# Hxyou/MSCLIP

Hardware: AMD Instinct MI355X
Metric: image-text pairs/sec ViT-B/32 bf16 (higher is better)
Workload: dtype bf16; 1 GPU; MS-CLIP-S b32-yfcc-msclips fwd + contrastive step (both towers, gather, logits, symmetric CE), per-GPU batch 512, 224x224 images + 77-token captions, random-init weights; per_gpu_batch=512, global_batch=512, parallelism=dp1, bn=eval (folded running statistics), rccl_ranks=1

## Files before the change

msclip_amd/csrc/attention.hip:

```cpp
#include <stdlib.h>
#include "common.h"
#include "plan.h"
#include "../../include/msclip_hip.h"

namespace {

template <int NT, bool CAUSAL, int WPB>
__global__ __launch_bounds__(WPB * 64) void attn_kernel(const bf16_t* __restrict__ qkv, bf16_t* __restrict__ out,
                                                   int nsamples, int Lfix, int H, int ldq, int ldo,
                                                   const int* __restrict__ cu, int pad_rows, const int* __restrict__ dims) {
  constexpr int KP = NT * 32;
  constexpr int KPS = KP + 8;
  extern __shared__ __attribute__((aligned(16))) bf16_t vt_all[];

  const int lane = threadIdx.x & 63;
  const int wave = __builtin_amdgcn_readfirstlane(threadIdx.x >> 6);
  const int pair = blockIdx.x * WPB + wave;
  if (pair >= nsamples * H) {
    const int r = pair - nsamples * H;
    if (dims) pad_rows = min(pad_rows, dims[4]);
    if (cu && r < pad_rows) {
      bf16_t* orow = out + (size_t)(cu[nsamples] + r) * ldo;
      for (int c = lane * 8; c < H * 64; c += 512) *(uint4*)(orow + c) = make_uint4(0, 0, 0, 0);
    }
    return;
  }
  const int b = pair / H, h = pair - b * H;
  bf16_t* vt = vt_all + wave * (64 * KPS);

  const int c0 = cu ? __builtin_amdgcn_readfirstlane(cu[b]) : b * Lfix;
  const int L = cu ? min(__builtin_amdgcn_readfirstlane(cu[b + 1]) - c0, KP) : Lfix;
  const size_t row0 = (size_t)c0;
  const bf16_t* qbase = qkv + row0 * ldq + h * 64;
  const bf16_t* kbase = qbase + H * 64;
  const bf16_t* vbase = qbase + 2 * H * 64;

  const int fr = lane & 31, fhi = lane >> 5;

  if constexpr (NT <= 3) {
    constexpr int NVI = KP / 8;
    uint4 vreg[NVI];
    {
      const int c = lane & 7;
#pragma unroll
      for (int i = 0; i < NVI; ++i) {
        const int key = i * 8 + (lane >> 3);
        vreg[i] = key < L ? *(const uint4*)(vbase + (size_t)key * ldq + c * 8) : make_uint4(0, 0, 0, 0);
      }
    }
    bf16x8 qf[NT][4], kf[NT][4];
#pragma unroll
    for (int t = 0; t < NT; ++t) {
      const int row = min(t * 32 + fr, L - 1);
      if (t * 32 < L) {
#pragma unroll
        for (int kk = 0; kk < 4; ++kk) {
          qf[t][kk] = *(const bf16x8*)(qbase + (size_t)row * ldq + (kk * 2 + fhi) * 8);
          kf[t][kk] = *(const bf16x8*)(kbase + (size_t)row * ldq + (kk * 2 + fhi) * 8);
        }
      } else {
#pragma unroll
        for (int kk = 0; kk < 4; ++kk) qf[t][kk] = kf[t][kk] = bf16x8{};
      }
    }
    {
      const int c = lane & 7;
#pragma unroll
      for (int i = 0; i < NVI; ++i) {
        const int key = i * 8 + (lane >> 3);
        const int w = key & 15;
        const int slot = (key & ~15) + (((w >> 2) & 1) << 3) + (w & 3) + ((w >> 3) << 2);
        bf16_t* dst = vt + (c * 8) * KPS + slot;
        const uint4 u = vreg[i];
        dst[0 * KPS] = (bf16_t)(u.x & 0xffff); dst[1 * KPS] = (bf16_t)(u.x >> 16);
        dst[2 * KPS] = (bf16_t)(u.y & 0xffff); dst[3 * KPS] = (bf16_t)(u.y >> 16);
        dst[4 * KPS] = (bf16_t)(u.z & 0xffff); dst[5 * KPS] = (bf16_t)(u.z >> 16);
        dst[6 * KPS] = (bf16_t)(u.w & 0xffff); dst[7 * KPS] = (bf16_t)(u.w >> 16);
      }
    }
    __builtin_amdgcn_wave_barrier();

#pragma unroll
    for (int qt = 0; qt < NT; ++qt) {
      if (qt * 32 < L) {
        const int nkt = CAUSAL ? (qt + 1) : NT;
        f32x16 s[NT];
#pragma unroll
        for (int kt = 0; kt < NT; ++kt) {
#pragma unroll
          for (int r = 0; r < 16; ++r) s[kt][r] = 0.f;
          if (kt < nkt && kt * 32 < L) {
#pragma unroll
            for (int kk = 0; kk < 4; ++kk)
              s[kt] = __builtin_amdgcn_mfma_f32_32x32x16_bf16(kf[kt][kk], qf[qt][kk], s[kt], 0, 0, 0);
          }
        }
        const int q = qt * 32 + fr;
        float mx = -INFINITY;
#pragma unroll
        for (int kt = 0; kt < NT; ++kt)
          if (kt < nkt) {
#pragma unroll
            for (int r = 0; r < 16; ++r) {
              const int key = kt * 32 + (r & 3) + 8 * (r >> 2) + 4 * fhi;
              const bool ok = key < L && (!CAUSAL || key <= q);
              s[kt][r] = ok ? s[kt][r] : -INFINITY;
              mx = fmaxf(mx, s[kt][r]);
            }
          }
        mx = fmaxf(mx, __shfl_xor(mx, 32, 64));
        float sum = 0.f;
#pragma unroll
        for (int kt = 0; kt < NT; ++kt)
          if (kt < nkt) {
#pragma unroll
            for (int r = 0; r < 16; ++r) {
              const float p = __expf(s[kt][r] - mx);
              s[kt][r] = p;
              sum += p;
            }
          }
        sum += __shfl_xor(sum, 32, 64);
        const float inv = 1.f / sum;
        f32x16 o[2];
#pragma unroll
        for (int dt = 0; dt < 2; ++dt)
#pragma unroll
          for (int r = 0; r < 16; ++r) o[dt][r] = 0.f;
#pragma unroll
        for (int kt = 0; kt < NT; ++kt) {
          if (kt < nkt && kt * 32 < L) {
#pragma unroll
            for (int half = 0; half < 2; ++half) {
              bf16x8 pf;
#pragma unroll
              for (int e = 0; e < 8; ++e) pf[e] = (__bf16)s[kt][half * 8 + e];
              const int st = kt * 2 + half;
#pragma unroll
              for (int dt = 0; dt < 2; ++dt) {
                const bf16x8 vf = *(const bf16x8*)(vt + (dt * 32 + fr) * KPS + st * 16 + fhi * 8);
                o[dt] = __builtin_amdgcn_mfma_f32_32x32x16_bf16(vf, pf, o[dt], 0, 0, 0);
              }
            }
          }
        }
        {
          bf16_t* orow = out + (row0 + min(q, L - 1)) * ldo + h * 64;
#pragma unroll
          for (int dt = 0; dt < 2; ++dt) {
            unsigned pk[4][2];
#pragma unroll
            for (int g = 0; g < 4; ++g) {
              pk[g][0] = pack_bf16x2(o[dt][g * 4 + 0] * inv, o[dt][g * 4 + 1] * inv);
              pk[g][1] = pack_bf16x2(o[dt][g * 4 + 2] * inv, o[dt][g * 4 + 3] * inv);
            }
#pragma unroll
            for (int s2 = 0; s2 < 2; ++s2) {
              const auto x = __builtin_amdgcn_permlane32_swap(pk[2 * s2][0], pk[2 * s2 + 1][0], false, false);
              const auto y = __builtin_amdgcn_permlane32_swap(pk[2 * s2][1], pk[2 * s2 + 1][1], false, false);
              if (q < L) *(uint4*)(orow + dt * 32 + s2 * 16 + fhi * 8) = make_uint4(x[0], y[0], x[1], y[1]);
            }
          }
        }
      }
    }
    return;
  }

  {
    const int c = lane & 7;
#pragma unroll 2
    for (int k0 = 0; k0 < KP; k0 += 8) {
      const int key = k0 + (lane >> 3);
      uint4 u = make_uint4(0, 0, 0, 0);
      if (key < L) u = *(const uint4*)(vbase + (size_t)key * ldq + c * 8);
      const int w = key & 15;
      const int slot = (key & ~15) + (((w >> 2) & 1) << 3) + (w & 3) + ((w >> 3) << 2);
      bf16_t* dst = vt + (c * 8) * KPS + slot;
      dst[0 * KPS] = (bf16_t)(u.x & 0xffff); dst[1 * KPS] = (bf16_t)(u.x >> 16);
      dst[2 * KPS] = (bf16_t)(u.y & 0xffff); dst[3 * KPS] = (bf16_t)(u.y >> 16);
      dst[4 * KPS] = (bf16_t)(u.z & 0xffff); dst[5 * KPS] = (bf16_t)(u.z >> 16);
      dst[6 * KPS] = (bf16_t)(u.w & 0xffff); dst[7 * KPS] = (bf16_t)(u.w >> 16);
    }
  }
  __builtin_amdgcn_s_waitcnt(0xc07f);
  __builtin_amdgcn_wave_barrier();

  for (int qt = 0; qt < NT; ++qt) {
    if (qt * 32 >= L) break;
    const int qrow = min(qt * 32 + fr, L - 1);
    bf16x8 qf[4];
#pragma unroll
    for (int kk = 0; kk < 4; ++kk) qf[kk] = *(const bf16x8*)(qbase + (size_t)qrow * ldq + (kk * 2 + fhi) * 8);

    const int nkt = CAUSAL ? (qt + 1) : NT;
    f32x16 s[NT];
#pragma unroll
    for (int kt = 0; kt < NT; ++kt) {
#pragma unroll
      for (int r = 0; r < 16; ++r) s[kt][r] = 0.f;
      if (kt < nkt && kt * 32 < L) {
        const int krow = min(kt * 32 + fr, L - 1);
#pragma unroll
        for (int kk = 0; kk < 4; ++kk) {
          const bf16x8 kf = *(const bf16x8*)(kbase + (size_t)krow * ldq + (kk * 2 + fhi) * 8);
          s[kt] = __builtin_amdgcn_mfma_f32_32x32x16_bf16(kf, qf[kk], s[kt], 0, 0, 0);
        }
      }
    }

    const int q = qt * 32 + fr;
    float mx = -INFINITY;
#pragma unroll
    for (int kt = 0; kt < NT; ++kt)
#pragma unroll
      for (int r = 0; r < 16; ++r) {
        const int key = kt * 32 + (r & 3) + 8 * (r >> 2) + 4 * fhi;
        const bool ok = key < L && (!CAUSAL || key <= q) && kt < nkt;
        s[kt][r] = ok ? s[kt][r] : -INFINITY;
        mx = fmaxf(mx, s[kt][r]);
      }
    mx = fmaxf(mx, __shfl_xor(mx, 32, 64));
    float sum = 0.f;
#pragma unroll
    for (int kt = 0; kt < NT; ++kt)
#pragma unroll
      for (int r = 0; r < 16; ++r) {
        const float p = __expf(s[kt][r] - mx);
        s[kt][r] = p;
        sum += p;
      }
    sum += __shfl_xor(sum, 32, 64);
    const float inv = 1.f / sum;

    f32x16 o[2];
#pragma unroll
    for (int dt = 0; dt < 2; ++dt)
#pragma unroll
      for (int r = 0; r < 16; ++r) o[dt][r] = 0.f;
#pragma unroll
    for (int kt = 0; kt < NT; ++kt) {
      if (kt < nkt && kt * 32 < L) {
#pragma unroll
        for (int half = 0; half < 2; ++half) {
          bf16x8 pf;
#pragma unroll
          for (int e = 0; e < 8; ++e) pf[e] = (__bf16)s[kt][half * 8 + e];
          const int st = kt * 2 + half;
#pragma unroll
          for (int dt = 0; dt < 2; ++dt) {
            const bf16x8 vf = *(const bf16x8*)(vt + (dt * 32 + fr) * KPS + st * 16 + fhi * 8);
            o[dt] = __builtin_amdgcn_mfma_f32_32x32x16_bf16(vf, pf, o[dt], 0, 0, 0);
          }
        }
      }
    }

    if (q < L) {
      bf16_t* orow = out + (row0 + q) * ldo + h * 64;
#pragma unroll
      for (int dt = 0; dt < 2; ++dt)
#pragma unroll
        for (int g = 0; g < 4; ++g) {
          uint2 v;
          v.x = pack_bf16x2(o[dt][g * 4 + 0] * inv, o[dt][g * 4 + 1] * inv);
          v.y = pack_bf16x2(o[dt][g * 4 + 2] * inv, o[dt][g * 4 + 3] * inv);
          *(uint2*)(orow + dt * 32 + g * 8 + fhi * 4) = v;
        }
    }
  }
}

template <int NT, bool CAUSAL>
__global__ __launch_bounds__(256, 2) void attn_wg_kernel(const bf16_t* __restrict__ qkv, bf16_t* __restrict__ out,
                                                      int nsamples, int L, int H, int ldq, int ldo) {
  constexpr int KP = NT * 32;
  constexpr int KPS = KP + 8;
  constexpr int KROW = 72;
  __shared__ __attribute__((aligned(16))) bf16_t kl[KP * KROW];
  __shared__ __attribute__((aligned(16))) bf16_t vt[64 * KPS];

  const int tid = threadIdx.x, lane = tid & 63;
  const int wave = __builtin_amdgcn_readfirstlane(tid >> 6);
  const int pair = blockIdx.x;
  const int b = pair / H, h = pair - b * H;
  const size_t row0 = (size_t)b * L;
  const bf16_t* qbase = qkv + row0 * ldq + h * 64;
  const bf16_t* kbase = qbase + H * 64;
  const bf16_t* vbase = qbase + 2 * H * 64;
  const int fr = lane & 31, fhi = lane >> 5;

  auto load_q = [&](int qt, bf16x8 (&qf)[4]) {
    const int qrow = min(qt * 32 + fr, L - 1);
#pragma unroll
    for (int kk = 0; kk < 4; ++kk) {
      const bf16_t* p = qbase + (size_t)qrow * ldq + (kk * 2 + fhi) * 8;
      asm volatile("global_load_dwordx4 %0, %1, off" : "=&v"(qf[kk]) : "v"(p));
    }
  };
  bf16x8 qcur[4], qnext[4];
#pragma unroll
  for (int kk = 0; kk < 4; ++kk) qcur[kk] = qnext[kk] = bf16x8{};
  if (wave * 32 < L) load_q(wave, qcur);

  {
    const int c = tid & 7;
    uint4 ku[NT], vu[NT];
#pragma unroll
    for (int i = 0; i < NT; ++i) {
      const int key = (tid >> 3) + 32 * i;
      const int kc = min(key, L - 1);
      ku[i] = *(const uint4*)(kbase + (size_t)kc * ldq + c * 8);
      vu[i] = *(const uint4*)(vbase + (size_t)kc * ldq + c * 8);
    }
#pragma unroll
    for (int i = 0; i < NT; ++i)
      if ((tid >> 3) + 32 * i >= L) ku[i] = vu[i] = make_uint4(0, 0, 0, 0);
#pragma unroll
    for (int i = 0; i < NT; ++i) {
      const int key = (tid >> 3) + 32 * i;
      *(uint4*)(kl + key * KROW + c * 8) = ku[i];
      const int w = key & 15;
      const int slot = (key & ~15) + (((w >> 2) & 1) << 3) + (w & 3) + ((w >> 3) << 2);
      bf16_t* dst = vt + (c * 8) * KPS + slot;
      dst[0 * KPS] = (bf16_t)(vu[i].x & 0xffff); dst[1 * KPS] = (bf16_t)(vu[i].x >> 16);
      dst[2 * KPS] = (bf16_t)(vu[i].y & 0xffff); dst[3 * KPS] = (bf16_t)(vu[i].y >> 16);
      dst[4 * KPS] = (bf16_t)(vu[i].z & 0xffff); dst[5 * KPS] = (bf16_t)(vu[i].z >> 16);
      dst[6 * KPS] = (bf16_t)(vu[i].w & 0xffff); dst[7 * KPS] = (bf16_t)(vu[i].w >> 16);
    }
  }
  asm volatile("s_waitcnt vmcnt(0)" : "+v"(qcur[0]), "+v"(qcur[1]), "+v"(qcur[2]), "+v"(qcur[3])::"memory");
  __syncthreads();

  for (int qt = wave; qt < NT && qt * 32 < L; qt += 4) {
    const bool more = (qt + 4) < NT && (qt + 4) * 32 < L;
    if (more) load_q(qt + 4, qnext);
    const int nkt = CAUSAL ? (qt + 1) : NT;
    f32x16 s[NT];
    if constexpr (!CAUSAL) {
      bf16x8 kf[2][4];
#pragma unroll
      for (int kk = 0; kk < 4; ++kk) kf[0][kk] = *(const bf16x8*)(kl + fr * KROW + (kk * 2 + fhi) * 8);
#pragma unroll
      for (int kt = 0; kt < NT; ++kt) {
        if (kt + 1 < NT) {
#pragma unroll
          for (int kk = 0; kk < 4; ++kk)
            kf[(kt + 1) & 1][kk] = *(const bf16x8*)(kl + ((kt + 1) * 32 + fr) * KROW + (kk * 2 + fhi) * 8);
        }
#pragma unroll
        for (int r = 0; r < 16; ++r) s[kt][r] = 0.f;
        __builtin_amdgcn_sched_barrier(0);
#pragma unroll
        for (int kk = 0; kk < 4; ++kk) s[kt] = __builtin_amdgcn_mfma_f32_32x32x16_bf16(kf[kt & 1][kk], qcur[kk], s[kt], 0, 0, 0);
        __builtin_amdgcn_sched_barrier(0);
      }
    } else {
#pragma unroll
      for (int kt = 0; kt < NT; ++kt) {
#pragma unroll
        for (int r = 0; r < 16; ++r) s[kt][r] = 0.f;
        if (kt < nkt && kt * 32 < L) {
#pragma unroll
          for (int kk = 0; kk < 4; ++kk) {
            const bf16x8 kf = *(const bf16x8*)(kl + (kt * 32 + fr) * KROW + (kk * 2 + fhi) * 8);
            s[kt] = __builtin_amdgcn_mfma_f32_32x32x16_bf16(kf, qcur[kk], s[kt], 0, 0, 0);
          }
        }
      }
    }
    const int q = qt * 32 + fr;
    float mx = -INFINITY;
#pragma unroll
    for (int kt = 0; kt < NT; ++kt) {
      const bool inside = kt * 32 + 32 <= L && (!CAUSAL || kt < qt) && kt < nkt;
      if (inside) {
#pragma unroll
        for (int r = 0; r < 16; ++r) mx = fmaxf(mx, s[kt][r]);
      } else {
#pragma unroll
        for (int r = 0; r < 16; ++r) {
          const int key = kt * 32 + (r & 3) + 8 * (r >> 2) + 4 * fhi;
          const bool ok = key < L && (!CAUSAL || key <= q) && kt < nkt;
          s[kt][r] = ok ? s[kt][r] : -INFINITY;
          mx = fmaxf(mx, s[kt][r]);
        }
      }
    }
    mx = fmaxf(mx, __shfl_xor(mx, 32, 64));
    const float mxl = mx * 1.44269504f;
    float sum = 0.f;
#pragma unroll
    for (int kt = 0; kt < NT; ++kt)
#pragma unroll
      for (int r = 0; r < 16; ++r) {
        const float p = __builtin_amdgcn_exp2f(fmaf(s[kt][r], 1.44269504f, -mxl));
        s[kt][r] = p;
        sum += p;
      }
    sum += __shfl_xor(sum, 32, 64);
    const float inv = 1.f / sum;
    f32x16 o[2];
#pragma unroll
    for (int dt = 0; dt < 2; ++dt)
#pragma unroll
      for (int r = 0; r < 16; ++r) o[dt][r] = 0.f;
    if constexpr (!CAUSAL) {
      bf16x8 vf[2][2];
#pragma unroll
      for (int dt = 0; dt < 2; ++dt) vf[0][dt] = *(const bf16x8*)(vt + (dt * 32 + fr) * KPS + fhi * 8);
#pragma unroll
      for (int st = 0; st < 2 * NT; ++st) {
        if (st + 1 < 2 * NT) {
#pragma unroll
          for (int dt = 0; dt < 2; ++dt)
            vf[(st + 1) & 1][dt] = *(const bf16x8*)(vt + (dt * 32 + fr) * KPS + (st + 1) * 16 + fhi * 8);
        }
        bf16x8 pf;
#pragma unroll
        for (int e = 0; e < 8; ++e) pf[e] = (__bf16)s[st >> 1][(st & 1) * 8 + e];
        __builtin_amdgcn_sched_barrier(0);
#pragma unroll
        for (int dt = 0; dt < 2; ++dt) o[dt] = __builtin_amdgcn_mfma_f32_32x32x16_bf16(vf[st & 1][dt], pf, o[dt], 0, 0, 0);
        __builtin_amdgcn_sched_barrier(0);
      }
    } else {
#pragma unroll
      for (int kt = 0; kt < NT; ++kt) {
        if (kt < nkt && kt * 32 < L) {
#pragma unroll
          for (int half = 0; half < 2; ++half) {
            bf16x8 pf;
#pragma unroll
            for (int e = 0; e < 8; ++e) pf[e] = (__bf16)s[kt][half * 8 + e];
            const int st = kt * 2 + half;
#pragma unroll
            for (int dt = 0; dt < 2; ++dt) {
              const bf16x8 vf = *(const bf16x8*)(vt + (dt * 32 + fr) * KPS + st * 16 + fhi * 8);
              o[dt] = __builtin_amdgcn_mfma_f32_32x32x16_bf16(vf, pf, o[dt], 0, 0, 0);
            }
          }
        }
      }
    }
    {
      bf16_t* orow = out + (row0 + min(q, L - 1)) * ldo + h * 64;
#pragma unroll
      for (int dt = 0; dt < 2; ++dt) {
        unsigned pk[4][2];
#pragma unroll
        for (int g = 0; g < 4; ++g) {
          pk[g][0] = pack_bf16x2(o[dt][g * 4 + 0] * inv, o[dt][g * 4 + 1] * inv);
          pk[g][1] = pack_bf16x2(o[dt][g * 4 + 2] * inv, o[dt][g * 4 + 3] * inv);
        }
#pragma unroll
        for (int s2 = 0; s2 < 2; ++s2) {
          const auto x = __builtin_amdgcn_permlane32_swap(pk[2 * s2][0], pk[2 * s2 + 1][0], false, false);
          const auto y = __builtin_amdgcn_permlane32_swap(pk[2 * s2][1], pk[2 * s2 + 1][1], false, false);
          if (q < L) *(uint4*)(orow + dt * 32 + s2 * 16 + fhi * 8) = make_uint4(x[0], y[0], x[1], y[1]);
        }
      }
    }
    if (more) {
      asm volatile("s_waitcnt vmcnt(4)" : "+v"(qnext[0]), "+v"(qnext[1]), "+v"(qnext[2]), "+v"(qnext[3])::"memory");
#pragma unroll
      for (int kk = 0; kk < 4; ++kk) qcur[kk] = qnext[kk];
    }
  }
}

template <int NT>
int launch_wg(const void* qkv, void* out, int nsamples, int L, int H, int ldq, int ldo, int causal, hipStream_t st) {
  const int pairs = nsamples * H;
  if (causal)
    hipLaunchKernelGGL((attn_wg_kernel<NT, true>), dim3(pairs), dim3(256), 0, st, (const bf16_t*)qkv, (bf16_t*)out,
                       nsamples, L, H, ldq, ldo);
  else
    hipLaunchKernelGGL((attn_wg_kernel<NT, false>), dim3(pairs), dim3(256), 0, st, (const bf16_t*)qkv, (bf16_t*)out,
                       nsamples, L, H, ldq, ldo);
  return msclip_launch_status();
}

template <int MAXI>
__global__ __launch_bounds__(256) void attn_lastq_kernel(const bf16_t* __restrict__ qc, int ldqc, const bf16_t* __restrict__ kv,
                                                    int ldkv, bf16_t* __restrict__ out, int ldo, int nsamples, int L, int H,
                                                    const int* __restrict__ last_row, int row_base, const int* __restrict__ cu) {
  const int lane = threadIdx.x & 63;
  const int pair = blockIdx.x * 4 + (threadIdx.x >> 6);
  if (pair >= nsamples * H) return;
  const int b = pair / H, h = pair - b * H;
  const int row0 = row_base + (cu ? cu[b] : b * L);
  int nk = cu ? cu[b + 1] - cu[b] : (last_row ? last_row[b] - row0 + 1 : L);
  nk = min(max(nk, 1), L);
  const int g = lane >> 3, c = lane & 7;
  const bf16_t* kbase = kv + (size_t)row0 * ldkv + H * 64 + h * 64 + c * 8;
  const bf16_t* vbase = kbase + H * 64;
  float q8[8];
  unpack_bf16x8(*(const uint4*)(qc + (size_t)b * ldqc + h * 64 + c * 8), q8);
  float s[MAXI];
  float m = -INFINITY;
#pragma unroll
  for (int i = 0; i < MAXI; ++i) {
    const int key = i * 8 + g;
    float d = 0.f;
    if (key < nk) {
      float kf[8];
      unpack_bf16x8(*(const uint4*)(kbase + (size_t)key * ldkv), kf);
#pragma unroll
      for (int e = 0; e < 8; ++e) d = fmaf(q8[e], kf[e], d);
    }
    d += __shfl_xor(d, 1, 64);
    d += __shfl_xor(d, 2, 64);
    d += __shfl_xor(d, 4, 64);
    s[i] = key < nk ? d : -INFINITY;
    m = fmaxf(m, s[i]);
  }
  m = fmaxf(m, __shfl_xor(m, 8, 64));
  m = fmaxf(m, __shfl_xor(m, 16, 64));
  m = fmaxf(m, __shfl_xor(m, 32, 64));
  float sum = 0.f;
#pragma unroll
  for (int i = 0; i < MAXI; ++i) {
    const float p = i * 8 + g < nk ? __expf(s[i] - m) : 0.f;
    sum += p;
    s[i] = bf16_to_f32(f32_to_bf16(p));
  }
  sum += __shfl_xor(sum, 8, 64);
  sum += __shfl_xor(sum, 16, 64);
  sum += __shfl_xor(sum, 32, 64);
  float acc[8] = {0.f, 0.f, 0.f, 0.f, 0.f, 0.f, 0.f, 0.f};
#pragma unroll
  for (int i = 0; i < MAXI; ++i) {
    const int key = i * 8 + g;
    if (key < nk) {
      float vf[8];
      unpack_bf16x8(*(const uint4*)(vbase + (size_t)key * ldkv), vf);
#pragma unroll
      for (int e = 0; e < 8; ++e) acc[e] = fmaf(s[i], vf[e], acc[e]);
    }
  }
#pragma unroll
  for (int e = 0; e < 8; ++e) {
    acc[e] += __shfl_xor(acc[e], 8, 64);
    acc[e] += __shfl_xor(acc[e], 16, 64);
    acc[e] += __shfl_xor(acc[e], 32, 64);
  }
  if (g == 0) {
    const float r = 1.f / sum;
    uint4 o;
    o.x = pack_bf16x2(acc[0] * r, acc[1] * r);
    o.y = pack_bf16x2(acc[2] * r, acc[3] * r);
    o.z = pack_bf16x2(acc[4] * r, acc[5] * r);
    o.w = pack_bf16x2(acc[6] * r, acc[7] * r);
    *(uint4*)(out + (size_t)b * ldo + h * 64 + c * 8) = o;
  }
}

template <int NT>
int launch(const void* qkv, void* out, int nsamples, int L, int H, int ldq, int ldo, int causal, hipStream_t st,
           const int* cu = nullptr, int pad_rows = 0, const int* dims = nullptr) {
  constexpr int WPB = NT > 4 ? 2 : 4;
  const int pairs = nsamples * H + (cu ? pad_rows : 0);
  const int grid = (pairs + WPB - 1) / WPB;
  const size_t lds = WPB * 64 * (NT * 32 + 8) * sizeof(bf16_t);
  if (causal)
    hipLaunchKernelGGL((attn_kernel<NT, true, WPB>), dim3(grid), dim3(WPB * 64), lds, st, (const bf16_t*)qkv,
                       (bf16_t*)out, nsamples, L, H, ldq, ldo, cu, pad_rows, dims);
  else
    hipLaunchKernelGGL((attn_kernel<NT, false, WPB>), dim3(grid), dim3(WPB * 64), lds, st, (const bf16_t*)qkv,
                       (bf16_t*)out, nsamples, L, H, ldq, ldo, cu, pad_rows, dims);
  return msclip_launch_status();
}

}

extern "C" int msclip_attention(const void* qkv, void* out, int nsamples, int L, int heads, int ldq, int ldo,
                                int causal, void* stream) {
  MSCLIP_PLAN_HOOK(msclip_attention, stream, qkv, out, nsamples, L, heads, ldq, ldo, causal);
  if (!qkv || !out || nsamples <= 0 || L <= 0 || heads <= 0 || (ldq % 8) || (ldo % 8)) return MSCLIP_EINVAL;
  hipStream_t st = (hipStream_t)stream;
  if (L <= 64) return launch<2>(qkv, out, nsamples, L, heads, ldq, ldo, causal, st);
  if (L <= 96) return launch<3>(qkv, out, nsamples, L, heads, ldq, ldo, causal, st);
  if (L <= 224) {
    const char* old = getenv("MSCLIP_ATTN_WAVE");
    if (old && old[0] == '1') return launch<7>(qkv, out, nsamples, L, heads, ldq, ldo, causal, st);
    return launch_wg<7>(qkv, out, nsamples, L, heads, ldq, ldo, causal, st);
  }
  if (L <= 288) return launch_wg<9>(qkv, out, nsamples, L, heads, ldq, ldo, causal, st);
  return MSCLIP_EINVAL;
}

static int lastq_launch(const void* q, int ldqc, const void* qkv, int ldq, void* out, int ldo, int nsamples, int L, int heads,
                        const int* last_row, int row_base, const int* cu, void* stream) {
  if (!q || !qkv || !out || nsamples <= 0 || L <= 0 || L > 288 || heads <= 0 || (ldqc % 8) || (ldq % 8) || (ldo % 8) || ldo < heads * 64 || row_base < 0)
    return MSCLIP_EINVAL;
  const int grid = (nsamples * heads + 3) / 4;
  hipStream_t st = (hipStream_t)stream;
#define LASTQ(MAXI)                                                                                                            \
  hipLaunchKernelGGL(attn_lastq_kernel<MAXI>, dim3(grid), dim3(256), 0, st, (const bf16_t*)q, ldqc, (const bf16_t*)qkv, ldq,   \
                     (bf16_t*)out, ldo, nsamples, L, heads, last_row, row_base, cu)
  if (L <= 32) LASTQ(4);
  else if (L <= 64) LASTQ(8);
  else if (L <= 80) LASTQ(10);
  else if (L <= 128) LASTQ(16);
  else if (L <= 256) LASTQ(32);
  else LASTQ(36);
#undef LASTQ
  return msclip_launch_status();
}

extern "C" int msclip_attention_lastq(const void* q, int ldqc, const void* qkv, int ldq, void* out, int ldo, int nsamples, int L,
                                      int heads, const int* last_row, int row_base, void* stream) {
  MSCLIP_PLAN_HOOK(msclip_attention_lastq, stream, q, ldqc, qkv, ldq, out, ldo, nsamples, L, heads, last_row, row_base);
  return lastq_launch(q, ldqc, qkv, ldq, out, ldo, nsamples, L, heads, last_row, row_base, nullptr, stream);
}

extern "C" int msclip_attention_lastq_varlen(const void* q, int ldqc, const void* qkv, int ldq, void* out, int ldo, int nsamples,
                                             int Lmax, int heads, const int* cu, int row_base, void* stream) {
  MSCLIP_PLAN_HOOK(msclip_attention_lastq_varlen, stream, q, ldqc, qkv, ldq, out, ldo, nsamples, Lmax, heads, cu, row_base);
  if (!cu) return MSCLIP_EINVAL;
  return lastq_launch(q, ldqc, qkv, ldq, out, ldo, nsamples, Lmax, heads, nullptr, row_base, cu, stream);
}

extern "C" int msclip_attention_varlen(const void* qkv, void* out, const int* cu, int nsamples, int Lmax, int heads, int ldq,
                                       int ldo, int causal, int pad_rows, const int* dims, void* stream) {
  MSCLIP_PLAN_HOOK(msclip_attention_varlen, stream, qkv, out, cu, nsamples, Lmax, heads, ldq, ldo, causal, pad_rows, dims);
  if (!qkv || !out || !cu || nsamples <= 0 || Lmax <= 0 || Lmax > 96 || heads <= 0 || (ldq % 8) || (ldo % 8) || pad_rows < 0 ||
      pad_rows > 255)
    return MSCLIP_EINVAL;
  hipStream_t st = (hipStream_t)stream;
  if (Lmax <= 32) return launch<1>(qkv, out, nsamples, Lmax, heads, ldq, ldo, causal, st, cu, pad_rows, dims);
  if (Lmax <= 64) return launch<2>(qkv, out, nsamples, Lmax, heads, ldq, ldo, causal, st, cu, pad_rows, dims);
  return launch<3>(qkv, out, nsamples, Lmax, heads, ldq, ldo, causal, st, cu, pad_rows, dims);
}
```

Measured before the change: 50250 pairs/s.

## Add persistent pipelined attention kernel with transposed-LDS V reads

Adds a persistent attention kernel for short sequences (NT<=3). Each wave loops over (sample, head) pairs and prefetches the next pair's Q/K/V into registers while computing the current one. V is now stored row-major in a swizzled LDS layout and read back with ds_read_tr16 transpose loads, which removes the per-element scalar transposed LDS stores. With default settings this path runs for fixed-length (non-varlen) inputs; varlen inputs use the old kernel with the new V layout. The cost is more register pressure from holding two pairs' fragments, plus a grid sized from an occupancy query.

```diff
diff --git a/msclip_amd/csrc/attention.hip b/msclip_amd/csrc/attention.hip
--- a/msclip_amd/csrc/attention.hip
+++ b/msclip_amd/csrc/attention.hip
@@ -5,7 +5,19 @@
 
 namespace {
 
-template <int NT, bool CAUSAL, int WPB>
+typedef __attribute__((ext_vector_type(4))) __bf16 bf16x4v;
+__device__ __forceinline__ bf16x8 ld_tr8(const char* p0, const char* p1) {
+  const bf16x4v lo = __builtin_amdgcn_ds_read_tr16_b64_v4bf16((AS3 bf16x4v*)p0);
+  const bf16x4v hi = __builtin_amdgcn_ds_read_tr16_b64_v4bf16((AS3 bf16x4v*)p1);
+  return __builtin_shufflevector(lo, hi, 0, 1, 2, 3, 4, 5, 6, 7);
+}
+__device__ __forceinline__ int vrm_store_off(int lane) { return (lane >> 3) * 128 + (((lane & 7) << 4) ^ (((lane >> 4) & 1) << 6)); }
+__device__ __forceinline__ int vrm_read_off(int lane, int dt) {
+  const int q = (lane & 15) >> 2;
+  return (4 * (lane >> 5) + q) * 128 + ((dt ^ (q >> 1)) << 6) + (((lane >> 4) & 1) << 5) + ((lane & 3) << 3);
+}
+
+template <int NT, bool CAUSAL, int WPB, bool VTR = false>
 __global__ __launch_bounds__(WPB * 64) void attn_kernel(const bf16_t* __restrict__ qkv, bf16_t* __restrict__ out,
                                                    int nsamples, int Lfix, int H, int ldq, int ldo,
                                                    const int* __restrict__ cu, int pad_rows, const int* __restrict__ dims) {
@@ -26,7 +38,7 @@
     return;
   }
   const int b = pair / H, h = pair - b * H;
-  bf16_t* vt = vt_all + wave * (64 * KPS);
+  bf16_t* vt = vt_all + wave * (VTR ? KP * 64 : 64 * KPS);
 
   const int c0 = cu ? __builtin_amdgcn_readfirstlane(cu[b]) : b * Lfix;
   const int L = cu ? min(__builtin_amdgcn_readfirstlane(cu[b + 1]) - c0, KP) : Lfix;
@@ -63,7 +75,11 @@
         for (int kk = 0; kk < 4; ++kk) qf[t][kk] = kf[t][kk] = bf16x8{};
       }
     }
-    {
+    if constexpr (VTR) {
+      char* dst = (char*)vt + vrm_store_off(lane);
+#pragma unroll
+      for (int i = 0; i < NVI; ++i) *(uint4*)(dst + i * 1024) = vreg[i];
+    } else {
       const int c = lane & 7;
 #pragma unroll
       for (int i = 0; i < NVI; ++i) {
@@ -79,6 +95,7 @@
       }
     }
     __builtin_amdgcn_wave_barrier();
+    const char* vtr[2] = {(const char*)vt + vrm_read_off(lane, 0), (const char*)vt + vrm_read_off(lane, 1)};
 
 #pragma unroll
     for (int qt = 0; qt < NT; ++qt) {
@@ -138,7 +155,8 @@
               const int st = kt * 2 + half;
 #pragma unroll
               for (int dt = 0; dt < 2; ++dt) {
-                const bf16x8 vf = *(const bf16x8*)(vt + (dt * 32 + fr) * KPS + st * 16 + fhi * 8);
+                const bf16x8 vf = VTR ? ld_tr8(vtr[dt] + st * 2048, vtr[dt] + st * 2048 + 1024)
+                                      : *(const bf16x8*)(vt + (dt * 32 + fr) * KPS + st * 16 + fhi * 8);
                 o[dt] = __builtin_amdgcn_mfma_f32_32x32x16_bf16(vf, pf, o[dt], 0, 0, 0);
               }
             }
@@ -268,6 +286,183 @@
           *(uint2*)(orow + dt * 32 + g * 8 + fhi * 4) = v;
         }
     }
+  }
+}
+
+template <int NT, bool CAUSAL>
+__global__ __launch_bounds__(256, 2) void attn_pipe_kernel(const bf16_t* __restrict__ qkv, bf16_t* __restrict__ out,
+                                                           int nsamples, int Lfix, int H, int ldq, int ldo,
+                                                           const int* __restrict__ cu, int pad_rows, const int* __restrict__ dims) {
+  constexpr int KP = NT * 32, NVI = KP / 8;
+  extern __shared__ __attribute__((aligned(16))) bf16_t vt_all[];
+  const int lane = threadIdx.x & 63;
+  const int wave = __builtin_amdgcn_readfirstlane(threadIdx.x >> 6);
+  const int gw = blockIdx.x * 4 + wave, nw = gridDim.x * 4, npairs = nsamples * H;
+  if (cu) {
+    if (dims) pad_rows = min(pad_rows, dims[4]);
+    const int end = __builtin_amdgcn_readfirstlane(cu[nsamples]);
+    for (int r = gw; r < pad_rows; r += nw) {
+      bf16_t* orow = out + (size_t)(end + r) * ldo;
+      for (int c = lane * 8; c < H * 64; c += 512) *(uint4*)(orow + c) = make_uint4(0, 0, 0, 0);
+    }
+  }
+  if (gw >= npairs) return;
+  char* vt = (char*)vt_all + wave * (KP * 128);
+  char* vst = vt + vrm_store_off(lane);
+  const char* vtr[2] = {vt + vrm_read_off(lane, 0), vt + vrm_read_off(lane, 1)};
+  const int fr = lane & 31, fhi = lane >> 5;
+
+  uint4 vreg[NVI];
+  bf16x8 qf[NT][4], kf[NT][4];
+#pragma unroll
+  for (int t = 0; t < NT; ++t)
+#pragma unroll
+    for (int kk = 0; kk < 4; ++kk) qf[t][kk] = kf[t][kk] = bf16x8{};
+  auto locate = [&](int pair, int& h, int& c0, int& L) {
+    const int b = pair / H;
+    h = pair - b * H;
+    c0 = cu ? __builtin_amdgcn_readfirstlane(cu[b]) : b * Lfix;
+    L = cu ? min(__builtin_amdgcn_readfirstlane(cu[b + 1]) - c0, KP) : Lfix;
+  };
+  const unsigned vlane = (unsigned)((lane >> 3) * ldq + (lane & 7) * 8) * 2;
+  auto load_v = [&](const bf16_t* vbase, int L) {
+#pragma unroll
+    for (int i = 0; i < NVI; ++i) {
+      const char* grp = (const char*)vbase + (size_t)(i * 8) * ldq * 2;
+      vreg[i] = i * 8 + (lane >> 3) < L ? *(const uint4*)(grp + vlane) : make_uint4(0, 0, 0, 0);
+    }
+  };
+  auto load_frag = [&](bf16x8 (&f)[4], const bf16_t* base, int t, int L) {
+    if (t * 32 < L) {
+      const unsigned off = (unsigned)(min(t * 32 + fr, L - 1) * ldq + fhi * 8) * 2;
+#pragma unroll
+      for (int kk = 0; kk < 4; ++kk) f[kk] = *(const bf16x8*)((const char*)base + kk * 32 + off);
+    }
+  };
+
+  int pair = gw, h, c0, L;
+  locate(pair, h, c0, L);
+  {
+    const bf16_t* qbase = qkv + (size_t)c0 * ldq + h * 64;
+    load_v(qbase + 2 * H * 64, L);
+#pragma unroll
+    for (int t = 0; t < NT; ++t) {
+      load_frag(qf[t], qbase, t, L);
+      load_frag(kf[t], qbase + H * 64, t, L);
+    }
+  }
+  for (;;) {
+#pragma unroll
+    for (int i = 0; i < NVI; ++i) *(uint4*)(vst + i * 1024) = vreg[i];
+    const int pn = pair + nw;
+    const bool more = pn < npairs;
+    int hn = 0, c0n = 0, Ln = 0;
+    const bf16_t* qbn = qkv;
+    if (more) {
+      locate(pn, hn, c0n, Ln);
+      qbn = qkv + (size_t)c0n * ldq + hn * 64;
+      load_v(qbn + 2 * H * 64, Ln);
+    }
+    __builtin_amdgcn_wave_barrier();
+    const size_t row0 = (size_t)c0;
+
+#pragma unroll
+    for (int qt = 0; qt < NT; ++qt) {
+      const bool live = qt * 32 < L;
+      const int nkt = CAUSAL ? (qt + 1) : NT;
+      f32x16 s[NT];
+      if (live) {
+#pragma unroll
+        for (int kt = 0; kt < NT; ++kt) {
+#pragma unroll
+          for (int r = 0; r < 16; ++r) s[kt][r] = 0.f;
+          if (kt < nkt && kt * 32 < L) {
+#pragma unroll
+            for (int kk = 0; kk < 4; ++kk)
+              s[kt] = __builtin_amdgcn_mfma_f32_32x32x16_bf16(kf[kt][kk], qf[qt][kk], s[kt], 0, 0, 0);
+          }
+        }
+      }
+      __builtin_amdgcn_sched_barrier(0);
+      if (more) {
+        load_frag(qf[qt], qbn, qt, Ln);
+        if (qt == NT - 1) {
+#pragma unroll
+          for (int t = 0; t < NT; ++t) load_frag(kf[t], qbn + H * 64, t, Ln);
+        }
+      }
+      __builtin_amdgcn_sched_barrier(0);
+      if (live) {
+        const int q = qt * 32 + fr;
+        float mx = -INFINITY;
+#pragma unroll
+        for (int kt = 0; kt < NT; ++kt)
+          if (kt < nkt) {
+#pragma unroll
+            for (int r = 0; r < 16; ++r) {
+              const int key = kt * 32 + (r & 3) + 8 * (r >> 2) + 4 * fhi;
+              const bool ok = key < L && (!CAUSAL || key <= q);
+              s[kt][r] = ok ? s[kt][r] : -INFINITY;
+              mx = fmaxf(mx, s[kt][r]);
+            }
+          }
+        mx = fmaxf(mx, __shfl_xor(mx, 32, 64));
+        float sum = 0.f;
+#pragma unroll
+        for (int kt = 0; kt < NT; ++kt)
+          if (kt < nkt) {
+#pragma unroll
+            for (int r = 0; r < 16; ++r) {
+              const float p = __expf(s[kt][r] - mx);
+              s[kt][r] = p;
+              sum += p;
+            }
+          }
+        sum += __shfl_xor(sum, 32, 64);
+        const float inv = 1.f / sum;
+        f32x16 o[2];
+#pragma unroll
+        for (int dt = 0; dt < 2; ++dt)
+#pragma unroll
+          for (int r = 0; r < 16; ++r) o[dt][r] = 0.f;
+#pragma unroll
+        for (int kt = 0; kt < NT; ++kt) {
+          if (kt < nkt && kt * 32 < L) {
+#pragma unroll
+            for (int half = 0; half < 2; ++half) {
+              bf16x8 pf;
+#pragma unroll
+              for (int e = 0; e < 8; ++e) pf[e] = (__bf16)s[kt][half * 8 + e];
+              const int st = kt * 2 + half;
+#pragma unroll
+              for (int dt = 0; dt < 2; ++dt) {
+                const bf16x8 vf = ld_tr8(vtr[dt] + st * 2048, vtr[dt] + st * 2048 + 1024);
+                o[dt] = __builtin_amdgcn_mfma_f32_32x32x16_bf16(vf, pf, o[dt], 0, 0, 0);
+              }
+            }
+          }
+        }
+        char* orow = (char*)(out + row0 * ldo + h * 64) + (unsigned)(min(q, L - 1) * ldo + fhi * 8) * 2;
+#pragma unroll
+        for (int dt = 0; dt < 2; ++dt) {
+          unsigned pk[4][2];
+#pragma unroll
+          for (int g = 0; g < 4; ++g) {
+            pk[g][0] = pack_bf16x2(o[dt][g * 4 + 0] * inv, o[dt][g * 4 + 1] * inv);
+            pk[g][1] = pack_bf16x2(o[dt][g * 4 + 2] * inv, o[dt][g * 4 + 3] * inv);
+          }
+#pragma unroll
+          for (int s2 = 0; s2 < 2; ++s2) {
+            const auto x = __builtin_amdgcn_permlane32_swap(pk[2 * s2][0], pk[2 * s2 + 1][0], false, false);
+            const auto y = __builtin_amdgcn_permlane32_swap(pk[2 * s2][1], pk[2 * s2 + 1][1], false, false);
+            if (q < L) *(uint4*)(orow + (dt * 32 + s2 * 16) * 2) = make_uint4(x[0], y[0], x[1], y[1]);
+          }
+        }
+      }
+    }
+    if (!more) break;
+    __builtin_amdgcn_wave_barrier();
+    pair = pn; h = hn; c0 = c0n; L = Ln;
   }
 }
 
@@ -556,12 +751,67 @@
   }
 }
 
+static int attn_pipe_mode() {
+  static const int mode = [] {
+    const char* e = getenv("MSCLIP_ATTN_PIPE");
+    return e && e[0] >= '0' && e[0] <= '2' ? e[0] - '0' : -1;
+  }();
+  return mode;
+}
+static int attn_grid_cap() {
+  static const int cap = [] {
+    const char* e = getenv("MSCLIP_ATTN_GRID");
+    const int v = e ? atoi(e) : 0;
+    return v > 0 ? v : 0;
+  }();
+  return cap;
+}
+
+template <int NT>
+int launch_pipe(const void* qkv, void* out, int nsamples, int L, int H, int ldq, int ldo, int causal, hipStream_t st,
+                const int* cu, int pad_rows, const int* dims) {
+  const size_t lds = 4 * (NT * 32) * 128;
+  static int resident[MSCLIP_MAXDEV] = {};
+  const int di = msclip_dev_index();
+  int occ = di >= 0 ? resident[di] : 0;
+  if (!occ) {
+    if (hipOccupancyMaxActiveBlocksPerMultiprocessor(&occ, attn_pipe_kernel<NT, false>, 256, lds) != hipSuccess || occ <= 0) occ = 2;
+    if (di >= 0) resident[di] = occ;
+  }
+  const int units = max(nsamples * H, cu ? pad_rows : 0);
+  const int wgs = (units + 3) / 4, fit = msclip_device_cus() * occ;
+  const int rounds = (wgs + fit - 1) / fit;
+  int grid = (wgs + rounds - 1) / rounds;
+  if (attn_grid_cap()) grid = min(grid, attn_grid_cap());
+  if (causal)
+    hipLaunchKernelGGL((attn_pipe_kernel<NT, true>), dim3(grid), dim3(256), lds, st, (const bf16_t*)qkv, (bf16_t*)out, nsamples,
+                       L, H, ldq, ldo, cu, pad_rows, dims);
+  else
+    hipLaunchKernelGGL((attn_pipe_kernel<NT, false>), dim3(grid), dim3(256), lds, st, (const bf16_t*)qkv, (bf16_t*)out, nsamples,
+                       L, H, ldq, ldo, cu, pad_rows, dims);
+  return msclip_launch_status();
+}
+
 template <int NT>
 int launch(const void* qkv, void* out, int nsamples, int L, int H, int ldq, int ldo, int causal, hipStream_t st,
            const int* cu = nullptr, int pad_rows = 0, const int* dims = nullptr) {
   constexpr int WPB = NT > 4 ? 2 : 4;
   const int pairs = nsamples * H + (cu ? pad_rows : 0);
   const int grid = (pairs + WPB - 1) / WPB;
+  if constexpr (NT <= 3) {
+    const int mode = attn_pipe_mode();
+    if (mode == 1 || (mode < 0 && !cu)) return launch_pipe<NT>(qkv, out, nsamples, L, H, ldq, ldo, causal, st, cu, pad_rows, dims);
+    if (mode != 0) {
+      const size_t ldsv = WPB * (NT * 32) * 128;
+      if (causal)
+        hipLaunchKernelGGL((attn_kernel<NT, true, WPB, true>), dim3(grid), dim3(WPB * 64), ldsv, st, (const bf16_t*)qkv,
+                           (bf16_t*)out, nsamples, L, H, ldq, ldo, cu, pad_rows, dims);
+      else
+        hipLaunchKernelGGL((attn_kernel<NT, false, WPB, true>), dim3(grid), dim3(WPB * 64), ldsv, st, (const bf16_t*)qkv,
+                           (bf16_t*)out, nsamples, L, H, ldq, ldo, cu, pad_rows, dims);
+      return msclip_launch_status();
+    }
+  }
   const size_t lds = WPB * 64 * (NT * 32 + 8) * sizeof(bf16_t);
   if (causal)
     hipLaunchKernelGGL((attn_kernel<NT, true, WPB>), dim3(grid), dim3(WPB * 64), lds, st, (const bf16_t*)qkv,
```

Result: no change. 50570 pairs/s, median of 6 (+0.6%).
